# NVlabs/bayes-sim-ig

Hardware: AMD Instinct MI355X
Metric: summary_vectors_per_sec_in_fit (higher is better)
Workload: dtype f32; 1 GPU; cfg5: ShadowHand MDRFF-4096 K=4 D=32, summary_start (I=2310), 100000 pairs/GPU, reference chunk protocol: <=1000-pair chunks, summarizer + 100 Adam updates x minibatch 100 + 6 held-out evals per chunk; pairs_per_gpu=100000, parallelism=dp1, gradient_exchange=none, hip_graph=True

## Files before the change

### bayes_sim_ig_amd/csrc/estimator.hip

```cpp
#include "comm.h"
#include "gemm.h"
#include "head.h"
#include "persist.h"
#include "persist_mdnn.h"

#include <algorithm>
#include <chrono>
#include <cmath>
#include <cstdlib>
#include <cstring>
#include <new>

namespace bsig {

int adam_launch(float* p, const float* g, float* m, float* v, int64_t n, float lr,
                float beta1, float beta2, float eps, int64_t t, const float* dyn,
                hipStream_t st);
int colsum_launch(const float* x, int64_t ld, int64_t rows, int64_t cols, float* out,
                  void* workspace, size_t workspace_bytes, hipStream_t st);

constexpr int64_t kAlign = 4;

struct Layout {
  int n_layers;
// ... 269 lines not shown
    }
  }
  const float4 zero = make_float4(0.f, 0.f, 0.f, 0.f);
#pragma unroll
  for (int r = 0; r < 4; ++r)
    for (int64_t i = (int64_t)blockIdx.x * blockDim.x + threadIdx.x; i < z.n4[r];
         i += (int64_t)gridDim.x * blockDim.x)
      z.ptr[r][i] = zero;
}

__global__ void iota_mod_kernel(int32_t* out, int n, int mod) {
  for (int i = blockIdx.x * blockDim.x + threadIdx.x; i < n; i += gridDim.x * blockDim.x)
    out[i] = i % mod;
}

static int64_t count_evals(int64_t n_updates) {
  const int64_t every = std::max<int64_t>(n_updates / 5, 1);
  int64_t n = 0;
  for (int64_t it = 0; it < n_updates; ++it)
    if (it % every == 0 || it + 1 == n_updates) ++n;
  return n;
}

}

using namespace bsig;

struct bsig_fit_plan {
  bsig_mdn_cfg cfg;
  Layout L;
  int64_t batch, max_test, n_updates, n_evals;
  bool hoist;
  bool feat_cache;
  bool feat_unique;
  bool feats_preloaded;
  const float* ext_feats;
  int64_t feat_rows;
  int64_t max_train;
  bsig_fit_buffers buf;
  bool bound;
  int64_t norm_batch;
  size_t train_ws_bytes, test_ws_bytes, feats_bytes, big_gemm_ws_bytes, iota_bytes;
  bool use_graph, split_adam;

  PersistEngine eng;
  UGeom ug; MdnnGeom mg;
  bool eng_off;
  int dp_evals_done;
  bool resident_ran;
  bool adam_pending;
  hipStream_t cap_stream;
  hipGraphExec_t g_step, g_grad, g_apply, g_eval;
  bool graphs_ready;
  const float* graph_feats;
  hipGraphExec_t g_dp; const bsig_comm* g_dp_comm;
  int g_dp_state;
  char g_dp_error[200];
};

namespace bsig {

static size_t plan_ws_bytes(const bsig_fit_plan* p) {
  return p->train_ws_bytes + p->test_ws_bytes + p->feats_bytes + p->big_gemm_ws_bytes +
         p->iota_bytes + p->eng.workspace_bytes;
}

// ... 53 lines not shown
  PersistCommon c;
  c.y = b.y_train; c.ldy = b.ldy_train; c.ids = b.ids_table;
  c.params = b.params; c.exp_avg = b.exp_avg; c.exp_avg_sq = b.exp_avg_sq;
  c.state = b.state; c.train_loss = b.train_loss;
  c.workspace = m.persist_ws; c.workspace_bytes = p->eng.workspace_bytes;
  if (p->split_adam) {
    c.grads = b.grads; c.adam_pending = p->adam_pending ? 1 : 0;
    p->adam_pending = false;
  }
  if (xr) { c.xr_ready = xr->ready; c.xr_done = xr->done; c.xr_base = xr->base; c.n_total = n; }
  if (eval_total > 0) {
    c.do_eval = 1; c.n_total = eval_total; c.eval_every = std::max(eval_total / 5, 1);
    c.n_test = (int)b.n_test;
    c.y_test = b.y_test; c.ldy_test = b.ldy_test; c.test_loss = b.test_loss;
  }
  c.hy.lr = p->cfg.lr; c.hy.beta1 = p->cfg.beta1; c.hy.beta2 = p->cfg.beta2;
  c.hy.adam_eps = p->cfg.adam_eps; c.hy.eps_noise = p->cfg.head.eps_noise;
  c.hy.min_weight = p->cfg.head.min_weight; c.hy.ll_limit = p->cfg.head.ll_limit;
  c.hy.norm_batch = p->norm_batch;
  if (engine(p) == 1) {
    PersistBuffers pb;
    static_cast<PersistCommon&>(pb) = c;
    pb.feats = m.feats; pb.ld_feats = p->cfg.rff_feats;
    pb.feat_ids = p->feat_unique ? b.ids_table : nullptr;
    pb.w_off = p->L.head_w_off; pb.b_off = p->L.head_b_off;
    pb.eval_row0 = p->feat_unique ? b.n_train : p->n_updates * p->batch;
    if (blk) {
      pb.feats = blk->feats; pb.ld_feats = blk->ld_feats; pb.feat_ids = blk->ids; pb.eval_row0 = 0;
      pb.y = blk->y; pb.ldy = blk->ldy; pb.ids = blk->ids;
      pb.train_loss = blk->train_loss; pb.test_loss = blk->test_loss;
      pb.y_test = blk->y; pb.ldy_test = blk->ldy; pb.n_test = blk->max_test;
      pb.chunks = blk->chunks; pb.n_chunks = blk->n_chunks;
    }
    return persist_run(persist_shape(p), p->ug, pb, n, st);
  }
  PersistMdnnBuffers pb;
  static_cast<PersistCommon&>(pb) = c;
  pb.x = b.x_train; pb.ldx = b.ldx_train;
  pb.x_kind = b.x_kind; pb.x_s = b.x_s; pb.x_a = b.x_a;
  pb.w1_off = p->L.w_off[0]; pb.b1_off = p->L.b_off[0];
  pb.w2_off = p->L.w_off[1]; pb.b2_off = p->L.b_off[1];
  pb.wh_off = p->L.head_w_off; pb.bh_off = p->L.head_b_off;
  pb.x_test = b.x_test; pb.ldx_test = b.ldx_test;
  pb.x_test_fac = b.x_test_factors; pb.ldx_test_fac = b.ldx_test_factors;
  return persist_mdnn_run(persist_mdnn_shape(p), p->mg, pb, n, st);
}

static Inputs train_inputs(const bsig_fit_plan* p, const PlanMem& m) {
  const bsig_fit_buffers& b = p->buf;
  Inputs in;
  in.dyn = b.state + ST_STEP; in.dyn_stride = p->batch;
  in.rff_coeff = b.rff_coeff; in.ld_coeff = b.ld_coeff; in.rff_offset = b.rff_offset;
  if (p->hoist) {
    in.x = m.feats; in.ldx = p->cfg.rff_feats; in.is_feat = true;
    if (p->feat_unique) in.rows = b.ids_table;
  }
  else { in.x = b.x_train; in.ldx = b.ldx_train; in.rows = b.ids_table; }
  return in;
}

static Inputs eval_inputs(const bsig_fit_plan* p, const PlanMem& m) {
  const bsig_fit_buffers& b = p->buf;
  Inputs in;
  in.rff_coeff = b.rff_coeff; in.ld_coeff = b.ld_coeff; in.rff_offset = b.rff_offset;
  if (p->hoist) {
    in.x = m.feats; in.ldx = p->cfg.rff_feats; in.is_feat = true;
// ... 223 lines not shown
                                  int64_t max_train_rows, int64_t max_test_rows,
                                  int64_t n_updates, int plan_flags, bsig_fit_plan** plan) {
  BSIG_REQUIRE(cfg && plan && batch >= 1 && max_train_rows >= 0 && max_test_rows >= 0 &&
               n_updates >= 0, "fit_create: bad args");
  bsig_fit_plan* p = new (std::nothrow) bsig_fit_plan();
  BSIG_REQUIRE(p, "fit_create: out of memory");
  std::memset(p, 0, sizeof(*p));
  p->cfg = *cfg;
  const int rc = make_layout(cfg, &p->L);
  if (rc != BSIG_OK) { delete p; return rc; }
  p->batch = batch; p->max_test = max_test_rows; p->norm_batch = batch;
  p->n_updates = n_updates; p->n_evals = count_evals(n_updates);
  Scratch s;
  carve(cfg, p->L, batch, nullptr, &s); p->train_ws_bytes = s.total_bytes;
  carve(cfg, p->L, std::max<int64_t>(max_test_rows, 1), nullptr, &s);
  p->test_ws_bytes = s.total_bytes;
  p->max_train = max_train_rows;
  const auto set = [](const char* name) { const char* e = getenv(name); return e && e[0] == '1'; };
  p->feat_cache = !set("BSIG_NO_FEAT_CACHE");
  if (!p->feat_cache) max_train_rows = 0;
  p->feat_rows = (max_train_rows > 0 ? std::min(n_updates * batch, max_train_rows)
                                     : n_updates * batch) + max_test_rows;
  const size_t feats = (size_t)p->feat_rows * (size_t)std::max(cfg->rff_feats, 0) * sizeof(float);
  p->hoist = cfg->rff_feats > 0 && n_updates > 0 && feats <= ((size_t)4 << 30) && !set("BSIG_NO_RFF_HOIST");
  if (!((plan_flags & BSIG_PLAN_NO_PERSISTENT) || set("BSIG_NO_PERSISTENT"))) {
    if (p->hoist && p->L.n_layers == 0 && cfg->head.full_cov == 0)
      persist_resolve(persist_shape(p), &p->ug, &p->eng);
    else if (cfg->rff_feats == 0 && p->L.n_layers == 2 && n_updates > 0)
      persist_mdnn_resolve(persist_mdnn_shape(p), &p->mg, &p->eng);
  }
  if (set("BSIG_NO_INKERNEL_EVAL")) p->eng.eval_single = p->eng.eval_dp = false;
  p->eng.block_launch = block_launch_resolved(p->eng.kind, p->eng.eval_single, set("BSIG_FIT_CHUNK_PER_LAUNCH"));
  p->eng.workspace_bytes = round_up<size_t>(p->eng.workspace_bytes, 256);
  if (p->hoist) {
    p->feats_bytes = round_up<size_t>(feats, 256);
    const int64_t mf = cfg->rff_cos_only ? cfg->rff_feats : cfg->rff_feats / 2;
    p->big_gemm_ws_bytes = round_up<size_t>(
        std::max(bsig_gemm_workspace_bytes(p->feat_rows - max_test_rows, mf, cfg->input_dim),
                 bsig_gemm_workspace_bytes(std::max<int64_t>(max_test_rows, 1), mf,
                                           cfg->input_dim)) + 256, 256);
  }
  *plan = p;
  return BSIG_OK;
}

extern "C" void bsig_fit_destroy(bsig_fit_plan* p) {
  if (!p) return;
  drop_graphs(p);
  if (p->cap_stream) (void)hipStreamDestroy(p->cap_stream);
  delete p;
}

extern "C" size_t bsig_fit_workspace_bytes(const bsig_fit_plan* p) {
  return p ? plan_ws_bytes(p) : 0;
}

extern "C" int bsig_fit_bind(bsig_fit_plan* p, const bsig_fit_buffers* b, int flags) {
  BSIG_REQUIRE(p && b, "fit_bind: null");
  BSIG_REQUIRE(b->params && b->grads && b->exp_avg && b->exp_avg_sq && b->state &&
               b->workspace && b->x_train && b->y_train && b->ids_table && b->train_loss &&
               b->test_loss, "fit_bind: null buffer");
  BSIG_REQUIRE(b->workspace_bytes >= plan_ws_bytes(p), "fit_bind: workspace %zu < %zu",
               b->workspace_bytes, plan_ws_bytes(p));
  BSIG_REQUIRE(!(p->max_train > 0 && b->n_train > p->max_train),
               "fit_bind: %lld training rows exceed the %lld the plan was sized for",
               (long long)b->n_train, (long long)p->max_train);
// ... 578 lines not shown
```

### bayes_sim_ig_amd/csrc/fit_persistent.hip

```cpp
#include "persist.h"

#include <algorithm>
#include <cstdlib>

#include "head_device.h"
#include "persist_device.h"

namespace bsig {

constexpr int kUT = 512;
constexpr int kUSteps = 18;
constexpr int kUGroup = 6;
constexpr int kUMT = 7;
constexpr int kULds = 160 * 1024;
constexpr int kUProf = 8;
constexpr int kUFP = 116;

struct UArgs {
  int B, Bp, MT;
  int Fdim, KS, ksteps, KB, WP;
  int Nh, NhP, D, K;
  int n_blocks, k_slices, G, T, n_owner, R;
  int n_updates, xs_floats;
  int fast_rows;
  const float* feats; int64_t ld_feats; const int32_t* feat_ids;
  const float* y; int64_t ldy; const int32_t* ids;
  float* params; float* m1; float* m2; int64_t w_off, b_off;
  int32_t* state; float* train_loss;
  double lr, beta1, beta2;
  float adam_eps, eps_noise, min_w, ll_limit, inv_norm;
  float* slabs; float* d_out; float* e_out; unsigned* flag_fwd; unsigned long long* gran;
  unsigned long long* gran_rep;
  float* grads; int adam_pending; int quad_ok;
  unsigned* xr_ready; const unsigned* xr_done; unsigned* xr_count; unsigned xr_base;
  int do_eval, eval_every, n_total, n_test, eval_passes, NE, RE;
  int64_t eval_row0;
  const float* y_test; int64_t ldy_test;
  float* test_loss;
  float* eval_slabs;
  unsigned* flag_eval;
  unsigned long long* gran_eval;
  long long* prof;
  int prof_t0;
  const bsig_fit_chunk* chunks; int n_chunks;
};

struct UCk {
  int step0, n_updates, n_total, eval_every, do_eval;
  unsigned ubase, evbase;
  uint64_t seed, rng_ctr0;
};
__device__ __forceinline__ int u_uniform(int v) { return __builtin_amdgcn_readfirstlane(v); }
__device__ __forceinline__ int64_t u_uniform(int64_t v) {
  return (int64_t)(((uint64_t)(uint32_t)u_uniform((int)((uint64_t)v >> 32)) << 32) | (uint32_t)u_uniform((int)(uint64_t)v));
}
__device__ __forceinline__ void u_chunk_load(const UArgs& p, int c, UCk& k) {
  if (p.chunks == nullptr) {
    k.step0 = p.state[0]; k.n_updates = p.n_updates; k.n_total = p.n_total; k.eval_every = p.eval_every;
    k.do_eval = p.do_eval; k.ubase = 0u; k.evbase = 0u;
    k.seed = reinterpret_cast<const uint64_t*>(p.state + 8)[0];
    k.rng_ctr0 = reinterpret_cast<const uint64_t*>(p.state + 8)[1];
    return;
  }
  const bsig_fit_chunk& e = p.chunks[c];
  k.step0 = 0; k.n_updates = u_uniform(e.n_updates); k.n_total = k.n_updates; k.eval_every = u_uniform(e.eval_every);
  k.do_eval = 1; k.ubase = (unsigned)u_uniform(e.upd_base); k.evbase = (unsigned)u_uniform(e.eval_base);
  k.seed = (uint64_t)u_uniform((int64_t)e.seed); k.rng_ctr0 = (uint64_t)u_uniform((int64_t)e.rng_ctr0);
}

struct UEval {
  int n_test, passes; int64_t row0;
  const float* y_test; int64_t ldy_test;
  float* out;
  unsigned gidx;
  uint64_t seed, stream;
};
__device__ __forceinline__ UEval u_eval_of(const UArgs& p, int c, int e) {
  UEval v;
  int every, n_total, step0;
  uint64_t ctr0;
  if (p.chunks == nullptr) {
    v.n_test = p.n_test; v.row0 = p.eval_row0; v.y_test = p.y_test; v.ldy_test = p.ldy_test; v.out = nullptr;
    v.gidx = (unsigned)e; every = p.eval_every; n_total = p.n_total; step0 = p.state[0];
    v.seed = reinterpret_cast<const uint64_t*>(p.state + 8)[0];
    ctr0 = reinterpret_cast<const uint64_t*>(p.state + 8)[1];
  } else {
    const bsig_fit_chunk& k = p.chunks[c];
    v.n_test = u_uniform(k.n_test); v.row0 = u_uniform(k.row0) + u_uniform(k.n_train);
    v.y_test = p.y + v.row0 * p.ldy; v.ldy_test = p.ldy; v.out = p.test_loss + u_uniform(k.test_slot) + e;
    v.gidx = (unsigned)u_uniform(k.eval_base) + (unsigned)e; every = u_uniform(k.eval_every);
    n_total = u_uniform(k.n_updates); step0 = 0;
    v.seed = (uint64_t)u_uniform((int64_t)k.seed); ctr0 = (uint64_t)u_uniform((int64_t)k.rng_ctr0);
  }
  v.passes = (v.n_test + p.B - 1) / p.B;
  const int at = min(e * every + 1, n_total);
  const int ev0 = p.do_eval || p.chunks ? (step0 == 0 ? 0 : (step0 - 1) / every + 1) : 0;
  v.stream = ctr0 + (uint64_t)(at - step0) + (uint64_t)(e - ev0);
  return v;
}
__device__ __forceinline__ int u_last_eval(int n_total, int every) { return n_total <= 1 ? 0 : (n_total - 2) / every + 1; }

__device__ __forceinline__ f32x4 umfma(float a, float b, f32x4 c) {
  return __builtin_amdgcn_mfma_f32_16x16x4f32(a, b, c, 0, 0, 0);
}

struct URole { int tile, owner; };
__device__ __forceinline__ URole wg_role(int wg, int T, int G) {
  const int per = T >> 3, rem = T & 7, gq = G >> 3, gr = G & 7;
  const int x = wg & 7, j = wg >> 3;
  const int tiles_x = gq + (x < gr ? 1 : 0);
  URole r;
  if (j < tiles_x) {
    r.tile = x * gq + min(x, gr) + j;
    int rank = 0;
    for (int xx = 0; xx < 8; ++xx) {
      const int cnt = wg > xx ? (wg - xx + 7) >> 3 : 0;
      rank += min(cnt, gq + (xx < gr ? 1 : 0));
    }
    r.owner = (T - G) + rank;
  } else {
    r.tile = -1;
    r.owner = x * (per - gq) + min(x, rem) - min(x, gr) + (j - tiles_x);
  }
  return r;
}

__device__ __forceinline__ int u_rowpos(int b) { return (b & ~15) + ((b & 3) << 2) + ((b >> 2) & 3); }

__device__ __forceinline__ int u_evals_before(int s, int every) { return s == 0 ? 0 : (s - 1) / every + 1; }

#define BSIG_USTAMP(k)                                                           \
  do {                                                                           \
    if (p.prof && threadIdx.x == 0 && pt >= p.prof_t0 && pt < p.prof_t0 + kUProf)  \
      p.prof[((int64_t)wg * kUProf + pt - p.prof_t0) * 16 + (k)] = wall_clock64(); \
// ... 99 lines not shown
      for (int s0 = 0; s0 < p.ksteps; s0 += kUGroup) {
        f32x4 breg[kUGroup];
#pragma unroll
        for (int q = 0; q < kUGroup; ++q) {
          const int col = k0 + 16 * (s0 + q) + 4 * g4;
          const f32x4 v = *reinterpret_cast<const f32x4*>(src + min((int64_t)col, p.ld_feats - 4));
          const f32x4 zero = {0.f, 0.f, 0.f, 0.f};
          breg[q] = col < p.Fdim ? v : zero;
        }
#pragma unroll
        for (int q = 0; q < kUGroup; ++q) {
#pragma unroll
          for (int nt = 0; nt < NT; ++nt) {
            const f32x4 a4 = *reinterpret_cast<const f32x4*>(ap + nt * 16 * p.WP + 16 * (s0 + q));
            acc[nt] = umfma(a4[0], breg[q][0], acc[nt]);
            acc[nt] = umfma(a4[1], breg[q][1], acc[nt]);
            acc[nt] = umfma(a4[2], breg[q][2], acc[nt]);
            acc[nt] = umfma(a4[3], breg[q][3], acc[nt]);
          }
        }
      }
      if (16 * w + c16 < rows) {
        const __amdgpu_buffer_rsrc_t sr = xwg_buffer(
            p.eval_slabs + ((((int64_t)(ev.gidx % 3u) * p.eval_passes + pass) * p.k_slices + ks) * B) * NhP + n0);
#pragma unroll
        for (int nt = 0; nt < NT; ++nt)
          xwg_store4(sr, (16 * w + c16) * NhP + 16 * nt + 4 * g4, acc[nt][0], acc[nt][1], acc[nt][2], acc[nt][3]);
      }
    }
  }
  __builtin_amdgcn_s_waitcnt(0);
  __syncthreads();
  if (tid == 0) flag_raise(p.flag_eval, slot, ev.gidx + 1u);
}

__device__ __forceinline__ void u_owner_eval(const UArgs& p, float* XS, float* red, int eo, const UEval& ev,
                                             const HeadArgs& a) {
  int tid = threadIdx.x;
  asm volatile("" : "+v"(tid));
  const int lane = tid & 63, w = tid >> 6;
  const int B = p.B, Nh = p.Nh, NhP = p.NhP, D = p.D, K = p.K, DK = D * K;
  const int per_wave = Nh + D + 3 * K;
  int32_t* flagp = p.state + 2;
  const unsigned etag = ev.gidx + 1u;
  if (w == 0) flags_wait(p.flag_eval, p.G, etag, lane, flagp);
  __syncthreads();
  const int nr = eo < ev.n_test ? min(p.RE, (ev.n_test - eo + p.NE - 1) / p.NE) : 0;
  const float* ebase = p.eval_slabs + (int64_t)(ev.gidx % 3u) * p.eval_passes * p.k_slices * B * NhP;
  float eacc = 0.f;
  u_rows_sum(ebase,
             [&](int r) {
               const int erow = eo + p.NE * r, pass = erow / B, rb = erow - pass * B;
               return (pass * p.k_slices * B + rb) * NhP;
             },
             p.k_slices, B * NhP, nr, Nh, XS, per_wave, tid,
             [&](int col, float v) { if (col >= K + DK && col < K + 2 * DK) eacc += expf(v); });
  eacc = wave_sum_dpp(eacc);
  if (lane == 0) red[w] = eacc;
  __syncthreads();
  if (tid == 0) {
    float sx = 0.f;
    for (int q = 0; q < kUT / 64; ++q) sx += red[q];
    granule_publish(p.gran_eval, eo, etag, sx);
  }
  const int erow = eo + p.NE * w;
  const bool act = w < nr;
// ... 560 lines not shown
          for (int v = 0; v < 4; ++v)
            if (w + 8 * jj < p.KB) Wl[(16 * nt + 4 * g4 + v) * WP + 16 * (w + 8 * jj) + c16] = Wv[jj][nt][v];
    }
    if (ks == 0 && w >= 8 - NT && g4 == 0) {
#pragma unroll
      for (int nt = 0; nt < NT; ++nt) {
        if (w != 8 - NT + nt) continue;
        const int n = n0 + 16 * nt + c16;
        if (n < Nh) {
          bw[nt] = p.params[p.b_off + n];
          if (!fresh) { bm[nt] = p.m1[p.b_off + n]; bv[nt] = p.m2[p.b_off + n]; }
          if (pend) {
            bw[nt] = adam_bias(p.grads[p.b_off + n], bm[nt], bv[nt], bw[nt], pa0, pa1, ak);
            p.params[p.b_off + n] = bw[nt]; p.m1[p.b_off + n] = bm[nt]; p.m2[p.b_off + n] = bv[nt];
          }
        }
        biasl[16 * nt + c16] = bw[nt];
      }
    }
  }
  if (tid == 0)
    red[63] = (__hip_atomic_load(flagp, __ATOMIC_RELAXED, __HIP_MEMORY_SCOPE_AGENT) & 2) ? 1.f : 0.f;
  if (has_tile && p.MT < kUMT)
    for (int idx = tid; idx < p.KS * (kUFP / 4); idx += kUT) {
      const f32x4 zero = {0.f, 0.f, 0.f, 0.f};
      *reinterpret_cast<f32x4*>(Ft + 4 * idx) = zero;
    }

  UOwn o;
  u_own_init(p, o, own, true, XS, red, Ft, lane0);
  u_own_chunk(o, ck);
  const int eo = (own - p.n_owner + p.T) % p.T;
  const bool has_erow = p.do_eval && eo < p.NE;
  int pending_eval = -1, pending_chunk = 0;

  f32x4 Freg[kUSteps];
  {
    const f32x4 zero = {0.f, 0.f, 0.f, 0.f};
#pragma unroll
    for (int S = 0; S < kUSteps; ++S) Freg[S] = zero;
  }
  int64_t pf_row = 0;
  {
    const int c16_l = c16, g4_l = g4;
    if (p.n_updates > 0) { BSIG_U_ROWID(p.feat_ids, 0, step0) BSIG_U_PREFETCH() }
  }
  __syncthreads();

  for (int c = 0; c < n_chunks; ++c) {
  if (c > 0) {
    u_chunk_load(p, c, ck);
    u_own_chunk(o, ck);
#pragma unroll
    for (int jj = 0; jj < MAXBLK; ++jj)
#pragma unroll
      for (int nt = 0; nt < NT; ++nt)
#pragma unroll
        for (int v = 0; v < 4; ++v) { Mr[jj][nt][v] = 0.f; Vr[jj][nt][v] = 0.f; }
#pragma unroll
    for (int nt = 0; nt < NT; ++nt) { bm[nt] = 0.f; bv[nt] = 0.f; }
    b1t = 1.0; b2t = 1.0;
  }
  const int step0 = ck.step0;
  for (int t = 0; t < p.n_updates; ++t) {
    int tid_l = tid, c16_l = c16, g4_l = g4;
    asm volatile("" : "+v"(tid_l), "+v"(c16_l), "+v"(g4_l));
    const int step = step0 + t;
// ... 31 lines not shown
                acc[nt] = umfma(a4[0], b4[0], acc[nt]);
                acc[nt] = umfma(a4[1], b4[1], acc[nt]);
                acc[nt] = umfma(a4[2], b4[2], acc[nt]);
                acc[nt] = umfma(a4[3], b4[3], acc[nt]);
              }
              ftp[(16 * S + 0) * FP] = b4[0];
              ftp[(16 * S + 1) * FP] = b4[1];
              ftp[(16 * S + 2) * FP] = b4[2];
              ftp[(16 * S + 3) * FP] = b4[3];
            }
          }
        }
        BSIG_USTAMP(1);
        if (rok) {
          const __amdgpu_buffer_rsrc_t sr = xwg_buffer(p.slabs + (int64_t)ks * B * NhP + n0);
#pragma unroll
          for (int nt = 0; nt < NT; ++nt)
            xwg_store4(sr, (16 * w + c16_l) * NhP + 16 * nt + 4 * g4_l, acc[nt][0], acc[nt][1], acc[nt][2], acc[nt][3]);
        }
      }
      __builtin_amdgcn_s_waitcnt(0);
      __syncthreads();
      if (tid_l == 0) flag_raise(p.flag_fwd, slot, epoch);
      BSIG_USTAMP(3);
      if (t + 1 < p.n_updates || c + 1 < n_chunks) { BSIG_U_ROWID(p.feat_ids, 0, epoch) }
    }
    if (tid_l == 0)
      red[63] = (__hip_atomic_load(flagp, __ATOMIC_RELAXED, __HIP_MEMORY_SCOPE_AGENT) & 2) ? 1.f : 0.f;
    b1t *= p.beta1; b2t *= p.beta2;
    a0 = (float)(p.lr / (1.0 - b1t));
    a1 = (float)(1.0 / sqrt(1.0 - b2t));

    if (has_row) u_own_update(p, o, t, w, lane0, wg);
    if (__builtin_expect(pending_eval >= 0, 0)) {
      __syncthreads();
      if (has_erow) u_owner_eval(p, XS, red, eo, u_eval_of(p, pending_chunk, pending_eval), o.a);
      pending_eval = -1;
    }
    if (__builtin_expect(p.do_eval && (step > 0 ? (step - 1) % p.eval_every == 0 : c > 0), 0)) {
      pending_chunk = step > 0 ? c : c - 1;
      pending_eval = step > 0 ? u_evals_before(step, p.eval_every) - 1 : u_last_eval(p.n_updates, p.eval_every);
      u_tile_eval<NT>(p, Wl, biasl, slot, ks, n0, k0, u_eval_of(p, pending_chunk, pending_eval));
    }

    {
      int tid_l = tid, c16_l = c16, g4_l = g4;
      asm volatile("" : "+v"(tid_l), "+v"(c16_l), "+v"(g4_l));
      const int lane = tid_l & 63;
      if (t + 1 < p.n_updates || c + 1 < n_chunks) { BSIG_U_PREFETCH() }
      BSIG_USTAMP(2);
      if (w == 0) {
        unsigned long long* sug = gran_rep(p, 1, wg & 7);
        const int n_su = (p.T - p.G >= p.n_owner && u_fast_kind(p) != 0) ? p.n_owner * 2 * p.R : p.n_owner;
        granule_wait_one(sug, slot % n_su, tag + 2, flagp);
        const float su = granule_gather(sug, n_su, tag + 2, lane, flagp);
        if (lane == 0) red[62] = p.eps_noise != 0.f ? p.eps_noise / ((float)B * (float)DK) * su : 0.f;
      }
      __syncthreads();
      BSIG_USTAMP(10);
      {
        const float c = red[62];
        const int sg_lo = K + DK, sg_hi = K + 2 * DK;
        const bool any_e = c != 0.f && n0 + NBW > sg_lo && n0 < sg_hi;
        const __amdgpu_buffer_rsrc_t dr = xwg_buffer(p.d_out + n0), er = xwg_buffer(p.e_out + n0);
        constexpr int QN = NBW / 4;
        constexpr int total = 16 * kUMT * QN;
        for (int base = 0; base < total; base += 2 * kUT) {
          f32x4 q[2], e[2];
#pragma unroll
          for (int u = 0; u < 2; ++u) {
            const int idx = base + u * kUT + tid_l;
            const int b = idx / QN, c4 = (idx - b * QN) * 4;
            const bool ok = idx < total && b < B;
            const f32x4 zero = {0.f, 0.f, 0.f, 0.f};
            q[u] = ok ? xwg_load4(dr, b * NhP + c4) : zero;
            e[u] = ok && any_e ? xwg_load4(er, b * NhP + c4) : zero;
          }
#pragma unroll
          for (int u = 0; u < 2; ++u) {
            const int idx = base + u * kUT + tid_l;
            const int b = idx / QN, c4 = (idx - b * QN) * 4;
            if (idx < total) {
// ... 152 lines not shown
            const f32x4 zero = {0.f, 0.f, 0.f, 0.f};
#pragma unroll
            for (int nt = 0; nt < NT; ++nt)
              gq[nt] = j < xr_kb ? xwg_load4s(xr_rsrc, xr_col + 128 * jj < xr_cols ? xr_lane + jj * 512 + nt * xr_nt : -1, 0) : zero;
#pragma unroll
            for (int nt = 0; nt < NT; ++nt) {
              const f32x4 c = quad_transpose4(gq[nt][0], gq[nt][1], gq[nt][2], gq[nt][3], c16_l & 3);
#pragma unroll
              for (int v = 0; v < 4; ++v) gr[nt][v] = c[v];
            }
#pragma unroll
            for (int nt = 0; nt < NT; ++nt)
#pragma unroll
              for (int v = 0; v < 4; ++v) {
                float* wp = Wl + (16 * nt + 4 * g4_l + v) * WP + 16 * j + c16_l;
                *wp = adam_weight(gr[nt][v], Mr[jj][nt][v], Vr[jj][nt][v], *wp, a0, a1, ak);
              }
          }
        }
      }
      BSIG_USTAMP(8);
      lds_barrier();
      BSIG_USTAMP(12);
    }
  }
  }
  if constexpr (XR) {
    if (slot == 0 && tid == 0 &&
        (__hip_atomic_load(flagp, __ATOMIC_RELAXED, __HIP_MEMORY_SCOPE_AGENT) & 2))
      __hip_atomic_store(p.xr_ready, p.xr_base + (unsigned)p.n_total, __ATOMIC_RELAXED, __HIP_MEMORY_SCOPE_SYSTEM);
  }

  if (p.do_eval && !run_aborted(flagp, red, tid)) {
    if (pending_eval >= 0) {
      if (has_erow) u_owner_eval(p, XS, red, eo, u_eval_of(p, pending_chunk, pending_eval), o.a);
      pending_eval = -1;
    }
    if (ck.step0 + p.n_updates == p.n_total && (!DP || p.n_updates == 0)) {
      const UEval ev = u_eval_of(p, n_chunks - 1, u_evals_before(p.n_total - 1, p.eval_every));
      __syncthreads();
      u_tile_eval<NT>(p, Wl, biasl, slot, ks, n0, k0, ev);
      if (has_erow) u_owner_eval(p, XS, red, eo, ev, o.a);
    }
  }
  if (!DP && has_tile) {
#pragma unroll
    for (int jj = 0; jj < MAXBLK; ++jj)
#pragma unroll
      for (int nt = 0; nt < NT; ++nt)
#pragma unroll
        for (int v = 0; v < 4; ++v) {
          const int n = n0 + 16 * nt + 4 * g4 + v, kc = 16 * (w + 8 * jj) + c16;
          if (w + 8 * jj < p.KB && n < Nh && k0 + kc < p.Fdim) {
            const int64_t off = p.w_off + (int64_t)n * p.Fdim + k0 + kc;
            p.params[off] = Wl[(16 * nt + 4 * g4 + v) * WP + kc];
            p.m1[off] = Mr[jj][nt][v]; p.m2[off] = Vr[jj][nt][v];
          }
        }
    if (ks == 0 && w >= 8 - NT && g4 == 0) {
#pragma unroll
      for (int nt = 0; nt < NT; ++nt) {
        if (w != 8 - NT + nt) continue;
        const int n = n0 + 16 * nt + c16;
        if (n < Nh) { p.params[p.b_off + n] = bw[nt]; p.m1[p.b_off + n] = bm[nt]; p.m2[p.b_off + n] = bv[nt]; }
      }
    }
  }
  if (p.prof && p.n_updates > 0 && tid == 0) {
    __builtin_amdgcn_s_waitcnt(0);
// ... 5 lines not shown
    int32_t* st = p.state;
    reinterpret_cast<double*>(st + 12)[0] = b1t;
    reinterpret_cast<double*>(st + 12)[1] = b2t;
    reinterpret_cast<float*>(st)[4] = a0;
    reinterpret_cast<float*>(st)[5] = a1;
    int n_ev = 0;
    if (ck.do_eval) {
      n_ev = u_evals_before(step0 + ck.n_updates, ck.eval_every) - u_evals_before(step0, ck.eval_every);
      if (!DP && step0 + ck.n_updates == ck.n_total && (ck.n_total - 1) % ck.eval_every != 0) ++n_ev;
    }
    reinterpret_cast<uint64_t*>(st + 8)[0] = ck.seed;
    reinterpret_cast<uint64_t*>(st + 8)[1] = ck.rng_ctr0 + (uint64_t)(ck.n_updates + n_ev);
    st[0] = step0 + ck.n_updates;
  }
}

__device__ __forceinline__ void owner_only_workgroup(const UArgs& p, float* smem, const URole& role, int NBW, bool dp) {
  float* XS = smem + p.KS * kUFP + NBW * p.WP;
  float* red = XS + p.xs_floats;
  const int tid = threadIdx.x, lane0 = tid & 63;
  const int w = __builtin_amdgcn_readfirstlane(tid >> 6);
  const int wg = blockIdx.x;
  int32_t* flagp = p.state + 2;
  const int n_chunks = (dp || p.chunks == nullptr) ? 1 : p.n_chunks;
  UCk ck;
  u_chunk_load(p, 0, ck);
  UOwn o;
  u_own_init(p, o, role.owner, false, XS, red, smem, lane0);
  u_own_chunk(o, ck);
  const bool has_row = role.owner < p.n_owner;
  const int eo = (role.owner - p.n_owner + p.T) % p.T;
  const bool has_erow = p.do_eval && eo < p.NE;
  const int fk = u_fast_kind(p);
  int pending_eval = -1, pending_chunk = 0;
  for (int c = 0; c < n_chunks; ++c) {
  if (c > 0) {
    u_chunk_load(p, c, ck);
    u_own_chunk(o, ck);
  }
  for (int t = 0; t < p.n_updates; ++t) {
    const int step = o.step0 + t;
    [[maybe_unused]] const int pt = t + (int)ck.ubase;
    if (run_aborted(flagp, red, tid)) break;
    BSIG_USTAMP(0);
    if (has_row) {
      switch (fk) {
        case 4 * 8 + 1: u_own_update_fast<4, 1>(p, o, t, w, lane0, wg); break;
        case 4 * 8 + 2: u_own_update_fast<4, 2>(p, o, t, w, lane0, wg); break;
        case 4 * 8 + 4: u_own_update_fast<4, 4>(p, o, t, w, lane0, wg); break;
        case 8 * 8 + 1: u_own_update_fast<8, 1>(p, o, t, w, lane0, wg); break;
        case 8 * 8 + 2: u_own_update_fast<8, 2>(p, o, t, w, lane0, wg); break;
        case 8 * 8 + 4: u_own_update_fast<8, 4>(p, o, t, w, lane0, wg); break;
        case 16 * 8 + 1: u_own_update_fast<16, 1>(p, o, t, w, lane0, wg); break;
        case 16 * 8 + 2: u_own_update_fast<16, 2>(p, o, t, w, lane0, wg); break;
        case 16 * 8 + 4: u_own_update_fast<16, 4>(p, o, t, w, lane0, wg); break;
        default: u_own_update(p, o, t, w, lane0, wg); break;
      }
    }
    if (__builtin_expect(pending_eval >= 0, 0)) {
      __syncthreads();
      if (has_erow) u_owner_eval(p, XS, red, eo, u_eval_of(p, pending_chunk, pending_eval), o.a);
      pending_eval = -1;
    }
    if (__builtin_expect(p.do_eval && (step > 0 ? (step - 1) % p.eval_every == 0 : c > 0), 0)) {
      pending_chunk = step > 0 ? c : c - 1;
      pending_eval = step > 0 ? u_evals_before(step, p.eval_every) - 1 : u_last_eval(p.n_updates, p.eval_every);
    }
    __syncthreads();
  }
  }
  if (p.do_eval && !run_aborted(flagp, red, tid)) {
    if (pending_eval >= 0 && has_erow)
      u_owner_eval(p, XS, red, eo, u_eval_of(p, pending_chunk, pending_eval), o.a);
    if (ck.step0 + p.n_updates == p.n_total && (!dp || p.n_updates == 0)) {
      const UEval ev = u_eval_of(p, n_chunks - 1, u_evals_before(p.n_total - 1, p.eval_every));
      __syncthreads();
      if (has_erow) u_owner_eval(p, XS, red, eo, ev, o.a);
    }
  }
}

template <bool DP, int NT, bool XR = false>
__global__ __launch_bounds__(kUT) void linear_head_updates_kernel(UArgs p) {
  extern __shared__ __attribute__((aligned(16))) float smem[];
#ifndef BSIG_HOST_SAN_BUILD
  const URole role = wg_role(blockIdx.x, p.T, p.G);
  if (role.tile < 0) owner_only_workgroup(p, smem, role, 16 * NT, DP);
  else unified_workgroup<DP, NT, XR>(p, smem, role);
#endif
}

__global__ void spin_kernel(long long ticks, int* sink) {
  extern __shared__ float spin_lds[];
  spin_lds[threadIdx.x] = 1.f;
  const long long t0 = wall_clock64();
  while (wall_clock64() - t0 < ticks) __builtin_amdgcn_s_sleep(64);
  if (spin_lds[threadIdx.x] == 2.f) sink[0] = 1;
}
int debug_spin(int blocks, size_t lds_bytes, int ms, hipStream_t st) {
  BSIG_REQUIRE(blocks >= 1 && ms >= 0 && lds_bytes <= (size_t)kULds, "debug_spin: bad args");
  BSIG_HIP(hipFuncSetAttribute(reinterpret_cast<const void*>(spin_kernel),
                               hipFuncAttributeMaxDynamicSharedMemorySize, kULds));
  hipLaunchKernelGGL(spin_kernel, dim3(blocks), dim3(256), std::max<size_t>(lds_bytes, 1024), st,
                     (long long)ms * 100000LL , (int*)nullptr);
  BSIG_CHECK_LAUNCH("debug_spin");
  return BSIG_OK;
// ... 16 lines not shown
  g->KS = KS;
  g->ksteps = g->KB = KS / 16;
  if (g->ksteps > kUSteps || g->KB > 8 * max_blk) return false;
  g->WP = KS + 4;
  g->k_slices = ceil_div(s.feat_dim, KS);
  g->G = g->n_blocks * g->k_slices;
  if (g->G > kXwgMax) return false;
  const int spare = kXwgMax - g->G;
  bool mixed = false;
  static const bool force_mixed = [] { const char* e = getenv("BSIG_PERSIST_MIXED"); return e && e[0] == '1'; }();
  if (!force_mixed && spare >= s.batch) { g->R = 1; g->T = g->G + s.batch; }
  else if (!force_mixed && spare >= ceil_div(s.batch, 2)) { g->R = 2; g->T = g->G + ceil_div(s.batch, 2); }
  else {
    mixed = true;
    g->T = std::max(g->G, std::min(s.batch, kXwgMax));
    g->R = ceil_div(s.batch, std::min(g->T, s.batch));
    if (g->R > kUT / 64) return false;
  }
  g->n_owner = ceil_div(s.batch, g->R);
  g->eval_passes = s.max_test > 0 ? ceil_div(s.max_test, s.batch) : 0;
  g->NE = 1; g->RE = 1;
  if (g->eval_passes > 0) {
    const int idle = g->T - g->n_owner;
    const int re_all = ceil_div(s.max_test, g->T);
    const int re_idle = idle > 0 ? ceil_div(s.max_test, idle) : 1 << 20;
    if (re_idle <= kUT / 64 && re_idle <= 2 * re_all) { g->NE = idle; g->RE = re_idle; }
    else { g->NE = g->T; g->RE = re_all; }
    if (g->RE > kUT / 64) { g->eval_passes = 0; g->NE = 1; g->RE = 1; }
    else g->NE = std::min(g->NE, ceil_div(s.max_test, g->RE));
  }
  auto lds_of = [&] {
    g->xs_floats = (int)round_up(std::max(NBW * g->FP, std::max(g->R, g->RE) * g->per_wave), 4);
    g->lds = ((size_t)g->KS * g->FP + (size_t)NBW * g->WP + g->xs_floats + 64 + NBW) * sizeof(float);
  };
  lds_of();
  if (g->lds > (size_t)kULds && g->eval_passes > 0 && g->RE > g->R) {
    g->eval_passes = 0; g->NE = 1; g->RE = 1;
    lds_of();
  }
  if (g->lds > (size_t)kULds) return false;
  g->slab_floats = (size_t)g->k_slices * s.batch * g->NhP;
  g->dout_floats = (size_t)s.batch * g->NhP;
  g->eval_floats = (size_t)3 * g->eval_passes * g->slab_floats;
  const double mfma_us = 32.0 * (2.0 * 4 * g->ksteps * NT + 4.0 * kUMT * NT * ceil_div(g->KB, 4)) / 2200.0;
  const double tile_us = mixed ? (double)s.batch * KS * 4 / 20000.0 : 0.0;
  const double sum_us = 0.035 * g->k_slices * g->R;
  *cost = mfma_us + tile_us + sum_us;
  return true;
}

static bool u_geom(const PersistShape& s, UGeom* g) {
  if (s.batch < 1 || s.batch > 16 * kUMT || s.feat_dim < 4 || s.feat_dim % 4 != 0 || s.out_dim < 1 ||
      s.n_comp < 1 || s.n_comp > 64)
    return false;
  const int groups = 64 / s.n_comp;
  if (ceil_div(s.out_dim, groups) > kElemsPerLane) return false;
  bool found = false;
  double best = 0.0;
  static const int force_nt = [] { const char* e = getenv("BSIG_PERSIST_NT"); return e ? atoi(e) : 0; }();
  static const int force_ks = [] { const char* e = getenv("BSIG_PERSIST_KS"); return e ? atoi(e) : 0; }();
  for (int NT = 1; NT <= 2; ++NT)
    for (int groups6 = 1; groups6 <= kUSteps / kUGroup; ++groups6) {
      UGeom c;
      double cost = 0.0;
      if ((force_nt && NT != force_nt) || (force_ks && 16 * kUGroup * groups6 != force_ks)) continue;
      if (!u_geom_try(s, NT, 16 * kUGroup * groups6, &c, &cost)) continue;
      if (!found || cost < best) { *g = c; best = cost; found = true; }
    }
  return found;
}

int persist_geometry(const PersistShape& s, int32_t* out) {
  UGeom g;
  for (int i = 0; i < 16; ++i) out[i] = 0;
  if (!u_geom(s, &g)) return 0;
  const int32_t v[13] = {g.NT, g.KS, g.n_blocks, g.k_slices, g.G, g.T, g.n_owner, g.R, g.NE, g.RE,
                         g.eval_passes, (int32_t)g.lds, std::max(0, g.n_owner - (g.T - g.G))};
  for (int i = 0; i < 13; ++i) out[i] = v[i];
  return 1;
}

static int u_allow_dynamic_lds() {
  static bool done[64] = {};
  const void* kernels[6] = {reinterpret_cast<const void*>(linear_head_updates_kernel<false, 1>),
                            reinterpret_cast<const void*>(linear_head_updates_kernel<false, 2>),
                            reinterpret_cast<const void*>(linear_head_updates_kernel<true, 1>),
                            reinterpret_cast<const void*>(linear_head_updates_kernel<false, 1, true>),
                            reinterpret_cast<const void*>(linear_head_updates_kernel<true, 2>),
                            reinterpret_cast<const void*>(linear_head_updates_kernel<false, 2, true>)};
  return allow_dynamic_lds(done, kernels, 6, kULds);
}

template <int NT>
static bool u_can_host(const UGeom& g) {
  int dev = 0;
  hipDeviceProp_t prop;
  if (hipGetDevice(&dev) != hipSuccess || hipGetDeviceProperties(&prop, dev) != hipSuccess) return false;
  if (prop.multiProcessorCount < g.T || (size_t)prop.maxSharedMemoryPerMultiProcessor < g.lds) return false;
  int per_cu = 0;
  if (u_allow_dynamic_lds() != BSIG_OK ||
      hipOccupancyMaxActiveBlocksPerMultiprocessor(&per_cu, linear_head_updates_kernel<false, NT>, kUT, g.lds) != hipSuccess)
    return false;
  return per_cu >= 1;
}

static size_t u_data_bytes(const UGeom& g) {
  return round_up<size_t>((g.slab_floats + 2 * g.dout_floats + g.eval_floats) * sizeof(float), 256);
}
static size_t u_sync_bytes() { return 2 * kFlagArr * sizeof(unsigned) + (6 + 16) * kGranArr * 8 + 256; }

bool persist_resolve(const PersistShape& s, UGeom* g, PersistEngine* e) {
// ... 58 lines not shown
  }
  p.grads = b.grads; p.adam_pending = b.adam_pending;
  p.xr_ready = b.xr_ready; p.xr_done = b.xr_done; p.xr_base = b.xr_base;
  p.xr_count = reinterpret_cast<unsigned*>(reinterpret_cast<char*>(b.workspace) + u_data_bytes(g) + u_sync_bytes() - 256);
  p.feats = b.feats; p.ld_feats = b.ld_feats; p.feat_ids = b.feat_ids; p.y = b.y; p.ldy = b.ldy; p.ids = b.ids;
  p.params = b.params; p.m1 = b.exp_avg; p.m2 = b.exp_avg_sq; p.w_off = b.w_off; p.b_off = b.b_off;
  p.quad_ok = (p.w_off % 4 == 0 && p.Fdim % 4 == 0 &&
               ((reinterpret_cast<uintptr_t>(b.params) | reinterpret_cast<uintptr_t>(b.exp_avg) |
                 reinterpret_cast<uintptr_t>(b.exp_avg_sq) | reinterpret_cast<uintptr_t>(b.grads)) & 15) == 0) ? 1 : 0;
  p.state = b.state; p.train_loss = b.train_loss;
  const PersistHyper& hy = b.hy;
  p.lr = hy.lr; p.beta1 = hy.beta1; p.beta2 = hy.beta2;
  p.adam_eps = hy.adam_eps; p.eps_noise = hy.eps_noise; p.min_w = hy.min_weight;
  p.ll_limit = hy.ll_limit; p.inv_norm = 1.0f / (float)hy.norm_batch;
  char* base = reinterpret_cast<char*>(b.workspace);
  p.slabs = reinterpret_cast<float*>(base);
  p.d_out = p.slabs + g.slab_floats;
  p.e_out = p.d_out + g.dout_floats;
  p.eval_slabs = p.e_out + g.dout_floats;
  char* sync = base + u_data_bytes(g);
  p.flag_fwd = reinterpret_cast<unsigned*>(sync);
  p.flag_eval = p.flag_fwd + kFlagArr;
  p.gran = reinterpret_cast<unsigned long long*>(sync + 2 * kFlagArr * sizeof(unsigned));
  p.gran_eval = p.gran + 3 * kGranArr;
  p.gran_rep = p.gran + 6 * kGranArr;
  p.NE = g.NE; p.RE = g.RE;
  if (b.do_eval) {
    BSIG_REQUIRE(g.eval_passes > 0 && b.n_test >= 1 && b.n_test <= g.eval_passes * s.batch &&
                     b.n_test <= g.NE * g.RE && b.y_test && b.test_loss && b.eval_every >= 1 && b.n_total >= 1,
                 "persistent updates: in-launch evaluation not covered");
    p.do_eval = 1; p.eval_every = b.eval_every; p.n_total = b.n_total; p.n_test = b.n_test;
    p.eval_passes = ceil_div(b.n_test, s.batch); p.eval_row0 = b.eval_row0;
    p.y_test = b.y_test; p.ldy_test = b.ldy_test; p.test_loss = b.test_loss;
  }
  if (b.chunks) { p.chunks = b.chunks; p.n_chunks = b.n_chunks; }
  p.prof = reinterpret_cast<long long*>(persist_profile_buffer());
  if (p.prof) {
    const char* t0 = getenv("BSIG_PROF_T0");
    p.prof_t0 = t0 ? atoi(t0) : 0;
  }
  if (b.xr_ready && !p.n_total) p.n_total = n;
  return g.NT == 1 ? u_launch<1>(g, p, b.grads != nullptr, n, b.do_eval != 0, st)
                   : u_launch<2>(g, p, b.grads != nullptr, n, b.do_eval != 0, st);
}

}
```

### bayes_sim_ig_amd/csrc/persist.h

```cpp
#pragma once
#include "common.h"

namespace bsig {

struct PersistEngine {
  int kind = 0;
  bool streams = false;
  bool eval_single = false;
  bool eval_dp = false;
  bool block_launch = false;
  size_t workspace_bytes = 0;
};

inline bool block_launch_resolved(int kind, bool eval_single, bool forced_single) {
  return kind == 1 && eval_single && !forced_single;
}

struct PersistShape {
  int batch, feat_dim, out_dim, n_comp;
  int max_test = 0;
};

struct UGeom {
  int NT, Bp, MT, FP, KS, ksteps, KB, WP, Nh, NhP, n_blocks, k_slices, G, T, n_owner, R;
  int per_wave, xs_floats;
  int eval_passes, NE, RE;
  size_t lds, slab_floats, dout_floats, eval_floats;
};

struct PersistHyper {
  double lr, beta1, beta2; float adam_eps, eps_noise, min_weight, ll_limit;
  int64_t norm_batch;
};

struct PersistCommon {
  const float* y; int64_t ldy;
  const int32_t* ids;
  float* params; float* exp_avg; float* exp_avg_sq;
  int32_t* state;
  float* train_loss;
  void* workspace; size_t workspace_bytes;
  float* grads = nullptr; int adam_pending = 0;
  unsigned* xr_ready = nullptr; const unsigned* xr_done = nullptr; unsigned xr_base = 0;
  int do_eval = 0; int eval_every = 1; int n_total = 0; int n_test = 0;
  const float* y_test = nullptr; int64_t ldy_test = 0;
  float* test_loss = nullptr;
  PersistHyper hy;
};

struct PersistBuffers : PersistCommon {
  const float* feats; int64_t ld_feats;
  const int32_t* feat_ids;
  int64_t w_off, b_off;
  int64_t eval_row0 = 0;
  const bsig_fit_chunk* chunks = nullptr; int n_chunks = 1;
};

bool persist_resolve(const PersistShape& s, UGeom* g, PersistEngine* e);
struct ZeroRegion { void* ptr; size_t bytes; };
int persist_reset_regions(const UGeom& g, void* workspace, size_t workspace_bytes, ZeroRegion* regions);
int persist_run(const PersistShape& s, const UGeom& g, const PersistBuffers& b, int n, hipStream_t st);

int persist_geometry(const PersistShape& s, int32_t* out);

inline int allow_dynamic_lds(bool (&done)[64], const void* const* kernels, int n, int bytes) {
  int dev = 0;
  BSIG_HIP(hipGetDevice(&dev));
  if (done[dev & 63]) return BSIG_OK;
  for (int i = 0; i < n; ++i)
    BSIG_HIP(hipFuncSetAttribute(kernels[i], hipFuncAttributeMaxDynamicSharedMemorySize, bytes));
  done[dev & 63] = true;
  return BSIG_OK;
}

void persist_set_profile_buffer(void* buf);
int debug_spin(int blocks, size_t lds_bytes, int ms, hipStream_t st);
void* persist_profile_buffer();

}
```

Measured before the change: 567,000 pairs/s.

## Spread in-kernel held-out evaluation tiles across subsequent update steps

Instead of computing every held-out evaluation tile in the step where an eval becomes due, the persistent kernel copies the current weights into a spare LDS region and computes a few eval tiles per following update step. A packed state word tracks progress, and the owner reduction runs once all slices are done or the next eval arrives. The aim is to remove the stall that a full eval tile pass puts on the update pipeline by overlapping it with Adam steps. In exchange it uses extra LDS for the weight snapshot, which can lower occupancy, and adds more state and control flow to the kernel.

```diff
diff --git a/bayes_sim_ig_amd/csrc/estimator.hip b/bayes_sim_ig_amd/csrc/estimator.hip
--- a/bayes_sim_ig_amd/csrc/estimator.hip
+++ b/bayes_sim_ig_amd/csrc/estimator.hip
@@ -325,6 +325,7 @@
   int64_t batch, max_test, n_updates, n_evals;
   bool hoist;
   bool feat_cache;
+  bool eval_one_wait = false;
   bool feat_unique;
   bool feats_preloaded;
   const float* ext_feats;
@@ -444,6 +445,7 @@
       pb.y_test = blk->y; pb.ldy_test = blk->ldy; pb.n_test = blk->max_test;
       pb.chunks = blk->chunks; pb.n_chunks = blk->n_chunks;
     }
+    pb.eval_one_wait = p->eval_one_wait ? 1 : 0;
     return persist_run(persist_shape(p), p->ug, pb, n, st);
   }
   PersistMdnnBuffers pb;
@@ -733,6 +735,7 @@
   if (set("BSIG_NO_INKERNEL_EVAL")) p->eng.eval_single = p->eng.eval_dp = false;
   p->eng.block_launch = block_launch_resolved(p->eng.kind, p->eng.eval_single, set("BSIG_FIT_CHUNK_PER_LAUNCH"));
   p->eng.workspace_bytes = round_up<size_t>(p->eng.workspace_bytes, 256);
+  p->eval_one_wait = set("BSIG_EVAL_ONE_WAIT");
   if (p->hoist) {
     p->feats_bytes = round_up<size_t>(feats, 256);
     const int64_t mf = cfg->rff_cos_only ? cfg->rff_feats : cfg->rff_feats / 2;
diff --git a/bayes_sim_ig_amd/csrc/fit_persistent.hip b/bayes_sim_ig_amd/csrc/fit_persistent.hip
--- a/bayes_sim_ig_amd/csrc/fit_persistent.hip
+++ b/bayes_sim_ig_amd/csrc/fit_persistent.hip
@@ -14,6 +14,7 @@
 constexpr int kUMT = 7;
 constexpr int kULds = 160 * 1024;
 constexpr int kUProf = 8;
+constexpr int kUEvalTiles = 2;
 constexpr int kUFP = 116;
 
 struct UArgs {
@@ -34,6 +35,7 @@
   float* grads; int adam_pending; int quad_ok;
   unsigned* xr_ready; const unsigned* xr_done; unsigned* xr_count; unsigned xr_base;
   int do_eval, eval_every, n_total, n_test, eval_passes, NE, RE;
+  int eval_ms;
   int64_t eval_row0;
   const float* y_test; int64_t ldy_test;
   float* test_loss;
@@ -100,6 +102,16 @@
 }
 __device__ __forceinline__ int u_last_eval(int n_total, int every) { return n_total <= 1 ? 0 : (n_total - 2) / every + 1; }
 
+
+typedef long long uest_t;
+__device__ __forceinline__ uest_t u_est(int c, int e, int done) { return ((uest_t)c << 40) | ((uest_t)e << 16) | (uest_t)done; }
+__device__ __forceinline__ int u_est_chunk(uest_t s) { return (int)(s >> 40); }
+__device__ __forceinline__ int u_est_eval(uest_t s) { return (int)((s >> 16) & 0xffffff); }
+__device__ __forceinline__ int u_est_done(uest_t s) { return (int)(s & 0xffff); }
+__device__ __forceinline__ int u_eval_slices(const UArgs& p, const UEval& ev) {
+  return p.eval_ms > 0 ? (ev.passes * p.MT + p.eval_ms - 1) / p.eval_ms : 1;
+}
+
 __device__ __forceinline__ f32x4 umfma(float a, float b, f32x4 c) {
   return __builtin_amdgcn_mfma_f32_16x16x4f32(a, b, c, 0, 0, 0);
 }
@@ -265,6 +277,82 @@
   __builtin_amdgcn_s_waitcnt(0);
   __syncthreads();
   if (tid == 0) flag_raise(p.flag_eval, slot, ev.gidx + 1u);
+}
+
+template <int NT>
+__device__ __forceinline__ void u_tile_eval_slice(const UArgs& p, const float* Ws, const float* bs, int slot,
+                                                  int ks, int n0, int k0, const UEval& ev, int slice, bool last) {
+  int tid = threadIdx.x;
+  asm volatile("" : "+v"(tid));
+  const int lane = tid & 63, w = __builtin_amdgcn_readfirstlane(tid >> 6), c16 = lane & 15, g4 = lane >> 4;
+  const int B = p.B, NhP = p.NhP;
+  const int i = kUT / 64 - 1 - w;
+  const int unit = slice * p.eval_ms + i, pass = unit / p.MT, mt = unit - pass * p.MT;
+  const int rows = min(B, ev.n_test - pass * B);
+  if (i < p.eval_ms && pass < ev.passes && 16 * mt < rows) {
+    f32x4 acc[NT];
+#pragma unroll
+    for (int nt = 0; nt < NT; ++nt) {
+      const f32x4 zero = {0.f, 0.f, 0.f, 0.f};
+      acc[nt] = ks == 0 ? *reinterpret_cast<const f32x4*>(bs + 16 * nt + 4 * g4) : zero;
+    }
+    const int64_t r = ev.row0 + pass * B + min(16 * mt + c16, rows - 1);
+    const float* src = p.feats + r * p.ld_feats;
+    const float* ap = Ws + c16 * p.WP + 4 * g4;
+    f32x4 breg[2][kUGroup];
+#pragma unroll
+    for (int q = 0; q < kUGroup; ++q)
+      breg[0][q] = *reinterpret_cast<const f32x4*>(src + min((int64_t)(k0 + 16 * q + 4 * g4), p.ld_feats - 4));
+#pragma unroll
+    for (int G6 = 0; G6 < kUSteps / kUGroup; ++G6) {
+      if (kUGroup * G6 < p.ksteps) {
+        if (G6 + 1 < kUSteps / kUGroup && kUGroup * (G6 + 1) < p.ksteps) {
+#pragma unroll
+          for (int q = 0; q < kUGroup; ++q)
+            breg[(G6 + 1) & 1][q] = *reinterpret_cast<const f32x4*>(
+                src + min((int64_t)(k0 + 16 * (kUGroup * (G6 + 1) + q) + 4 * g4), p.ld_feats - 4));
+        }
+        __builtin_amdgcn_sched_barrier(0);
+#pragma unroll
+        for (int q = 0; q < kUGroup; ++q) {
+          const f32x4 zero = {0.f, 0.f, 0.f, 0.f};
+          const f32x4 b4 = k0 + 16 * (kUGroup * G6 + q) + 4 * g4 < p.Fdim ? breg[G6 & 1][q] : zero;
+#pragma unroll
+          for (int nt = 0; nt < NT; ++nt) {
+            const f32x4 a4 = *reinterpret_cast<const f32x4*>(ap + nt * 16 * p.WP + 16 * (kUGroup * G6 + q));
+            acc[nt] = umfma(a4[0], b4[0], acc[nt]);
+            acc[nt] = umfma(a4[1], b4[1], acc[nt]);
+            acc[nt] = umfma(a4[2], b4[2], acc[nt]);
+            acc[nt] = umfma(a4[3], b4[3], acc[nt]);
+          }
+        }
+        __builtin_amdgcn_sched_barrier(0);
+      }
+    }
+    if (16 * mt + c16 < rows) {
+      const __amdgpu_buffer_rsrc_t sr = xwg_buffer(
+          p.eval_slabs + ((((int64_t)(ev.gidx % 3u) * p.eval_passes + pass) * p.k_slices + ks) * B) * NhP + n0);
+#pragma unroll
+      for (int nt = 0; nt < NT; ++nt)
+        xwg_store4(sr, (16 * mt + c16) * NhP + 16 * nt + 4 * g4, acc[nt][0], acc[nt][1], acc[nt][2], acc[nt][3]);
+    }
+    __builtin_amdgcn_s_waitcnt(0);
+  }
+  if (last) {
+    __syncthreads();
+    if (tid == 0) flag_raise(p.flag_eval, slot, ev.gidx + 1u);
+  }
+}
+
+__device__ __forceinline__ void u_snapshot(const UArgs& p, const float* Wl, const float* biasl, float* Ws, int nbw) {
+  int tid = threadIdx.x;
+  asm volatile("" : "+v"(tid));
+  const int nq = nbw * p.WP / 4;
+  for (int idx = tid; idx < nq; idx += kUT)
+    *reinterpret_cast<f32x4*>(Ws + 4 * idx) = *reinterpret_cast<const f32x4*>(Wl + 4 * idx);
+  if (tid < nbw / 4)
+    *reinterpret_cast<f32x4*>(Ws + nbw * p.WP + 4 * tid) = *reinterpret_cast<const f32x4*>(biasl + 4 * tid);
+  __syncthreads();
 }
 
 __device__ __forceinline__ void u_owner_eval(const UArgs& p, float* XS, float* red, int eo, const UEval& ev,
@@ -891,7 +979,8 @@
   u_own_chunk(o, ck);
   const int eo = (own - p.n_owner + p.T) % p.T;
   const bool has_erow = p.do_eval && eo < p.NE;
-  int pending_eval = -1, pending_chunk = 0;
+  uest_t est = -1;
+  const bool spread = !DP && !XR && p.eval_ms > 0;
 
   f32x4 Freg[kUSteps];
   {
@@ -989,22 +1078,46 @@
     a1 = (float)(1.0 / sqrt(1.0 - b2t));
 
     if (has_row) u_own_update(p, o, t, w, lane0, wg);
-    if (__builtin_expect(pending_eval >= 0, 0)) {
+    const bool due = p.do_eval && (step > 0 ? (step - 1) % p.eval_every == 0 : c > 0);
+    bool pf_out = false;
+    if (__builtin_expect(est >= 0 || due, 0)) {
+      BSIG_USTAMP(6);
+      if (spread && (t + 1 < p.n_updates || c + 1 < n_chunks)) { BSIG_U_PREFETCH() pf_out = true; }
       __syncthreads();
-      if (has_erow) u_owner_eval(p, XS, red, eo, u_eval_of(p, pending_chunk, pending_eval), o.a);
-      pending_eval = -1;
-    }
-    if (__builtin_expect(p.do_eval && (step > 0 ? (step - 1) % p.eval_every == 0 : c > 0), 0)) {
-      pending_chunk = step > 0 ? c : c - 1;
-      pending_eval = step > 0 ? u_evals_before(step, p.eval_every) - 1 : u_last_eval(p.n_updates, p.eval_every);
-      u_tile_eval<NT>(p, Wl, biasl, slot, ks, n0, k0, u_eval_of(p, pending_chunk, pending_eval));
+      float* Ws = biasl + NBW;
+#pragma unroll 1
+      for (int rnd = 0; rnd < 2; ++rnd) {
+        if (rnd == 1) {
+          if (!due) break;
+          est = u_est(step > 0 ? c : c - 1,
+                      step > 0 ? u_evals_before(step, p.eval_every) - 1 : u_last_eval(p.n_updates, p.eval_every), 0);
+          if (spread) u_snapshot(p, Wl, biasl, Ws, NBW);
+        }
+        if (est < 0) continue;
+        const UEval ev = u_eval_of(p, u_est_chunk(est), u_est_eval(est));
+        const int ns = u_eval_slices(p, ev);
+        int done = u_est_done(est);
+        const bool finish = rnd == 0 && (due || done == ns);
+        const int upto = finish ? ns : done + 1;
+        for (; done < upto; ++done) {
+          if (spread) u_tile_eval_slice<NT>(p, Ws, Ws + NBW * WP, slot, ks, n0, k0, ev, done, done == ns - 1);
+          else u_tile_eval<NT>(p, Wl, biasl, slot, ks, n0, k0, ev);
+        }
+        if (finish) {
+          if (has_erow) u_owner_eval(p, XS, red, eo, ev, o.a);
+          est = -1;
+        } else {
+          est += 1;
+        }
+      }
+      BSIG_USTAMP(15);
     }
 
     {
       int tid_l = tid, c16_l = c16, g4_l = g4;
       asm volatile("" : "+v"(tid_l), "+v"(c16_l), "+v"(g4_l));
       const int lane = tid_l & 63;
-      if (t + 1 < p.n_updates || c + 1 < n_chunks) { BSIG_U_PREFETCH() }
+      if (!pf_out && (t + 1 < p.n_updates || c + 1 < n_chunks)) { BSIG_U_PREFETCH() }
       BSIG_USTAMP(2);
       if (w == 0) {
         unsigned long long* sug = gran_rep(p, 1, wg & 7);
@@ -1223,9 +1336,13 @@
   }
 
   if (p.do_eval && !run_aborted(flagp, red, tid)) {
-    if (pending_eval >= 0) {
-      if (has_erow) u_owner_eval(p, XS, red, eo, u_eval_of(p, pending_chunk, pending_eval), o.a);
-      pending_eval = -1;
+    if (est >= 0) {
+      const UEval ev = u_eval_of(p, u_est_chunk(est), u_est_eval(est));
+      const int ns = u_eval_slices(p, ev);
+      for (int done = u_est_done(est); spread && done < ns; ++done)
+        u_tile_eval_slice<NT>(p, biasl + NBW, biasl + NBW + NBW * WP, slot, ks, n0, k0, ev, done, done == ns - 1);
+      if (has_erow) u_owner_eval(p, XS, red, eo, ev, o.a);
+      est = -1;
     }
     if (ck.step0 + p.n_updates == p.n_total && (!DP || p.n_updates == 0)) {
       const UEval ev = u_eval_of(p, n_chunks - 1, u_evals_before(p.n_total - 1, p.eval_every));
@@ -1297,7 +1414,7 @@
   const int eo = (role.owner - p.n_owner + p.T) % p.T;
   const bool has_erow = p.do_eval && eo < p.NE;
   const int fk = u_fast_kind(p);
-  int pending_eval = -1, pending_chunk = 0;
+  uest_t est = -1;
   for (int c = 0; c < n_chunks; ++c) {
   if (c > 0) {
     u_chunk_load(p, c, ck);
@@ -1322,21 +1439,26 @@
         default: u_own_update(p, o, t, w, lane0, wg); break;
       }
     }
-    if (__builtin_expect(pending_eval >= 0, 0)) {
-      __syncthreads();
-      if (has_erow) u_owner_eval(p, XS, red, eo, u_eval_of(p, pending_chunk, pending_eval), o.a);
-      pending_eval = -1;
-    }
-    if (__builtin_expect(p.do_eval && (step > 0 ? (step - 1) % p.eval_every == 0 : c > 0), 0)) {
-      pending_chunk = step > 0 ? c : c - 1;
-      pending_eval = step > 0 ? u_evals_before(step, p.eval_every) - 1 : u_last_eval(p.n_updates, p.eval_every);
-    }
+    const bool due = p.do_eval && (step > 0 ? (step - 1) % p.eval_every == 0 : c > 0);
+    if (__builtin_expect(est >= 0, 0)) {
+      const UEval ev = u_eval_of(p, u_est_chunk(est), u_est_eval(est));
+      if (due || u_est_done(est) == u_eval_slices(p, ev)) {
+        __syncthreads();
+        if (has_erow) u_owner_eval(p, XS, red, eo, ev, o.a);
+        est = -1;
+      } else {
+        est += 1;
+      }
+    }
+    if (__builtin_expect(due, 0))
+      est = u_est(step > 0 ? c : c - 1,
+                  step > 0 ? u_evals_before(step, p.eval_every) - 1 : u_last_eval(p.n_updates, p.eval_every), 1);
     __syncthreads();
   }
   }
   if (p.do_eval && !run_aborted(flagp, red, tid)) {
-    if (pending_eval >= 0 && has_erow)
-      u_owner_eval(p, XS, red, eo, u_eval_of(p, pending_chunk, pending_eval), o.a);
+    if (est >= 0 && has_erow)
+      u_owner_eval(p, XS, red, eo, u_eval_of(p, u_est_chunk(est), u_est_eval(est)), o.a);
     if (ck.step0 + p.n_updates == p.n_total && (!dp || p.n_updates == 0)) {
       const UEval ev = u_eval_of(p, n_chunks - 1, u_evals_before(p.n_total - 1, p.eval_every));
       __syncthreads();
@@ -1419,6 +1541,9 @@
   auto lds_of = [&] {
     g->xs_floats = (int)round_up(std::max(NBW * g->FP, std::max(g->R, g->RE) * g->per_wave), 4);
     g->lds = ((size_t)g->KS * g->FP + (size_t)NBW * g->WP + g->xs_floats + 64 + NBW) * sizeof(float);
+    const size_t snap = ((size_t)NBW * g->WP + NBW) * sizeof(float);
+    g->snap = g->eval_passes > 0 && g->lds + snap <= (size_t)kULds ? 1 : 0;
+    if (g->snap) g->lds += snap;
   };
   lds_of();
   if (g->lds > (size_t)kULds && g->eval_passes > 0 && g->RE > g->R) {
@@ -1464,6 +1589,7 @@
   const int32_t v[13] = {g.NT, g.KS, g.n_blocks, g.k_slices, g.G, g.T, g.n_owner, g.R, g.NE, g.RE,
                          g.eval_passes, (int32_t)g.lds, std::max(0, g.n_owner - (g.T - g.G))};
   for (int i = 0; i < 13; ++i) out[i] = v[i];
+  out[14] = g.snap;
   return 1;
 }
 
@@ -1588,6 +1714,12 @@
     p.do_eval = 1; p.eval_every = b.eval_every; p.n_total = b.n_total; p.n_test = b.n_test;
     p.eval_passes = ceil_div(b.n_test, s.batch); p.eval_row0 = b.eval_row0;
     p.y_test = b.y_test; p.ldy_test = b.ldy_test; p.test_loss = b.test_loss;
+    if (g.snap && !b.eval_one_wait && !b.grads) {
+      const char* e = getenv("BSIG_EVAL_SLICE_TILES");
+      p.eval_ms = std::min(std::max(e ? atoi(e) : kUEvalTiles, 1), kUT / 64);
+      BSIG_REQUIRE(ceil_div(p.eval_passes * g.MT, p.eval_ms) < (1 << 16) && b.n_total < (1 << 24) && b.n_chunks < (1 << 22),
+                   "persistent updates: evaluation schedule out of range");
+    }
   }
   if (b.chunks) { p.chunks = b.chunks; p.n_chunks = b.n_chunks; }
   p.prof = reinterpret_cast<long long*>(persist_profile_buffer());
diff --git a/bayes_sim_ig_amd/csrc/persist.h b/bayes_sim_ig_amd/csrc/persist.h
--- a/bayes_sim_ig_amd/csrc/persist.h
+++ b/bayes_sim_ig_amd/csrc/persist.h
@@ -25,6 +25,7 @@
   int NT, Bp, MT, FP, KS, ksteps, KB, WP, Nh, NhP, n_blocks, k_slices, G, T, n_owner, R;
   int per_wave, xs_floats;
   int eval_passes, NE, RE;
+  int snap;
   size_t lds, slab_floats, dout_floats, eval_floats;
 };
 
@@ -54,6 +55,7 @@
   int64_t w_off, b_off;
   int64_t eval_row0 = 0;
   const bsig_fit_chunk* chunks = nullptr; int n_chunks = 1;
+  int eval_one_wait = 0;
 };
 
 bool persist_resolve(const PersistShape& s, UGeom* g, PersistEngine* e);
```

New measurement: 545,300 pairs/s. 0.962x the previous value.
